# homenc/HElib

Measured on AMD Instinct MI355X. Metric: ctxt_x_ctxt_mults_per_sec_incl_relinearize, higher is better.
Workload: dtype u64; 1 GPU; BGV m=32768 p=65537 bits=950 (L=16x60b, K=6x56b, 6 small primes, D=3): Ctxt::multiplyBy on FRESH ciphertexts = multLowLvl (bringToSet x2 + tensorProduct) + reLinearize (dropSmallAndSpecialPrimes + key switch), benchmarks/bgv_basic.cpp:144-165; added noise MEASURED as in the reference (device canonical-embedding norms, read back lazily); the loop is driven by the C++17 host (libhelib_amd_host.so); ; batch_per_gpu=128, pairs_all_ranks=128

## Files before the change

### helib_amd/csrc/engine.hip

```cpp
#include <hip/hip_runtime.h>

#include <cstdarg>
#include <cstdio>
#include <cstdlib>
#include <cstring>
#include <algorithm>
#include <chrono>
#include <map>
#include <mutex>
#include <string>
#include <unordered_set>
#include <vector>

#include "../../include/helib_amd.h"
#include "arena.h"
#include "prof.h"
#include "switches.h"
#include "dev_common.h"
#include "hostmath.h"
#include "bluestein.h"
#include "pfa_dev.h"
#include "rns_kernels.h"
#include "mfma_ext.h"
#include "rns_mfma_dev.h"
#include "norm_kernels.h"
#include "prg_kernels.h"

namespace hx {
hipError_t launch_ntt_pow2(int logn, bool inverse, const uint64_t* in, uint64_t* out,
                           const NttRows& rows, int nrows, int batch, const PrimeDev* primes,
                           const TW* tw_arena, hipStream_t st);
hipError_t launch_ntt_pow2_lazy_in(int logn, const uint64_t* in, uint64_t* out, const NttRows& rows, int nrows, int batch,
                                   const PrimeDev* primes, const TW* tw_arena, hipStream_t st);
hipError_t launch_keyswitch_last_pow2(int logn, int nd, const KsLastArgs& A, const RowMap2& map, const KsLastPlan& plan, int device,
                                      const PrimeDev* primes, const TW* tw_arena, hipStream_t st);
hipError_t launch_ntt_half15_fwd(bool lazy_in, const uint64_t* in, uint64_t* out, const NttRows& rows, int nrows, int batch,
                                 const PrimeDev* sub_primes, const TW* tw_arena, hipStream_t st);
hipError_t launch_moddown_pow2(int logn, const PolyBases& data, const PolyBases& out, int drop_row,
                               int drop_prime, const NttRows& keep, int nkeep, int batch,
                               const ModDownPrep& P, const ModDownApply& A, const PrimeDev* primes,
                               const TW* tw_arena, hipStream_t st);
hipError_t launch_moddown_prep_pow2(int logn, const PolyBases& polys, int drop_row, int drop_prime, int batch,
                                    const ModDownPrep& P, const PrimeDev* primes, const TW* tw_arena,
                                    hipStream_t st);
hipError_t launch_moddown_prep_multi_pow2(int logn, const PolyBases& polys, const PrepMulti& M, int ndrop, int batch,
                                          const ModDownPrep& P, const PrimeDev* primes, const TW* tw_arena,
                                          hipStream_t st);
hipError_t launch_moddown_apply_plain_pow2(int logn, const PolyBases& polys, const PolyBases& outs,
                                           const NttRows& keep, int nkeep, int batch, const ModDownApply& A,
                                           const PrimeDev* primes, const TW* tw_arena, hipStream_t st);
hipError_t launch_moddown_prep_multi_tensor_pow2(int logn, const TensorSrc& T, const PrepMulti& M, int ndrop, int batch,
                                                 const ModDownPrep& P, const PrimeDev* primes, const TW* tw_arena,
                                                 hipStream_t st);
hipError_t launch_moddown_apply_plain_tensor_pow2(int logn, const TensorSrc& T, const PolyBases& outs, const NttRows& keep,
                                                  int nkeep, int batch, const ModDownApply& A, const PrimeDev* primes,
                                                  const TW* tw_arena, hipStream_t st);
hipError_t launch_moddown_tensor_pow2(int logn, const TensorSrc& T, const PolyBases& outs, int drop_row, int drop_prime,
                                      const NttRows& keep, int nkeep, int batch, const ModDownPrep& P,
                                      const ModDownApply& A, const PrimeDev* primes, const TW* tw_arena, hipStream_t st);
hipError_t launch_ntt_inv_mul_pow2(int logn, const uint64_t* a, const uint64_t* b, uint64_t* out, const NttRows& rows,
                                   int nrows, int batch, const PrimeDev* primes, const TW* tw_arena, hipStream_t st);
hipError_t launch_conv_rows(int logn, const ConvRowArgs& A, const ConvRows& R, int nunits, const PrimeDev* cprimes,
                            const TW* tw_arena, hipStream_t st);
}

using hx::ExtArgs;
using hx::ExtPlanDev;
using hx::MAX_ROWS;
static constexpr int MAX_EXT_SRC = hx::EXT_MAXSRC;
using hx::ModDownApply;
using hx::ModDownPrep;
using hx::NttRows;
using hx::PolyBases;
using hx::PrimeDev;
using hx::RowMap;
using hx::RowMap2;
using hx::RowScalars;
using hx::TW;

static thread_local std::string g_err;
static int fail(int code, const char* fmt, ...)
{
  char buf[512];
  va_list ap;
  va_start(ap, fmt);
  vsnprintf(buf, sizeof buf, fmt, ap);
  va_end(ap);
  g_err = buf;
  return code;
}
#define HIPCHK(expr)                                                                     \
  do {                                                                                   \
    hipError_t _e = (expr);                                                              \
    if (_e != hipSuccess) {                                                              \
      (void)hipGetLastError();  \
      return fail(HX_ERR_DEVICE, "%s failed: %s (%s:%d)", #expr, hipGetErrorString(_e),  \
                  __FILE__, __LINE__);                                                   \
    }                                                                                    \
  } while (0)
#define CHK(expr)          \
  do {                     \
// ... 4306 lines not shown
    plan.fd[r] = (uint16_t)fd[r];
  }
  hx::KsLastArgs A;
  CHK(ks_fix_table(c, all, owner, digit_primes, &A.fix));
  A.dig_in = dig_in;
  A.dig_ev = dig_ev;
  A.kb = W->d_b;
  A.ka = W->d_a;
  A.out0 = out0;
  A.out1 = out1;
  A.own_src = own_src;
  A.acc0 = t0s ? t0s : out0;
  A.acc1 = t0s ? t1s : out1;
  A.scale_parts = t0s ? 1 : 0;
  A.nall = nall;
  A.wrows = (int)W->row_idx.size();
  A.batch = batch;
  hipError_t e = hx::launch_keyswitch_last_pow2(c->logn, ndig, A, map, plan, c->device, c->d_primes, c->d_tw, c->stream);
  if (e != hipSuccess)
    return fail(HX_ERR_DEVICE, "key-switch launch failed: %s", hipGetErrorString(e));
  return HX_OK;
}

extern "C" int hx_key_switch_digits(const hx_poly* digits, const hx_ksk* W, hx_poly* out0,
                                    hx_poly* out1)
{
  if (!digits || !W || !out0 || !out1)
    return fail(HX_ERR_INVALID, "null argument");
  hx_ctx* c = digits->ctx;
  CTX_ENTER(c);
  const int nall = out0->nrows();
  if (nall == 0 || out1->prime_idx != out0->prime_idx || out0->batch != digits->batch ||
      out1->batch != digits->batch)
    return fail(HX_ERR_PRIMESET, "Ctxt::addPart: ctxt has primes not in part");
  if (digits->nrows() % nall != 0 || digits->nrows() / nall > W->ndig || digits->nrows() == 0)
    return fail(HX_ERR_INVALID, "W must have as many columns as there are digits");
  const int ndig = digits->nrows() / nall;
  for (int d = 0; d < ndig; d++)
    for (int r = 0; r < nall; r++)
      if (digits->prime_idx[(size_t)d * nall + r] != out0->prime_idx[r])
        return fail(HX_ERR_PRIMESET, "digit rows do not match the ciphertext's primes");
  OWN(out0);
  OWN(out1);
  return keyswitch_launch(c, digits->d, W, out0->prime_idx, digits->batch, out0->d, out1->d, nall,
                          nullptr, nullptr, nullptr, ndig);
}

static int relin_core(hx_ctx* c, const uint64_t* t2e, const std::vector<int>& own,
                      const std::vector<int>& all, const hx_ksk* W, const int* dig_idx,
                      const int* dig_off, int ndig, int batch, uint64_t* out0, uint64_t* out1,
                      const uint64_t* t0s = nullptr, const uint64_t* t1s = nullptr, const hx::TensorSrc* ts = nullptr)
{
  const int L = (int)own.size(), nall = (int)all.size();
  const size_t rw = (size_t)batch * c->phim;
  CHK(ensure_scratch(c, 2, (size_t)L * rw));
  if (ts) {
    NttRows nr;
    for (int r = 0; r < L; r++) {
      nr.row[r] = (uint16_t)r;
      nr.prime[r] = (uint16_t)own[r];
    }
    hipError_t e = hx::launch_ntt_inv_mul_pow2(c->logn, ts->a1, ts->b1, c->scratch[2], nr, L, batch, c->d_primes,
                                               c->d_tw, c->stream);
    if (e != hipSuccess)
      return fail(HX_ERR_DEVICE, "NTT launch failed: %s", hipGetErrorString(e));
  } else {
    std::vector<std::pair<int, int>> rows;
    for (int r = 0; r < L; r++)
      rows.emplace_back(r, own[r]);
    CHK(ntt_list(c, t2e, c->scratch[2], rows, batch, true));
  }
  CHK(ensure_scratch(c, 1, (size_t)ndig * nall * rw));
  std::vector<int> owner;
  {
    int rc = break_digits_fused(c, c->scratch[2], own, dig_idx, dig_off, ndig, all, c->scratch[1],
                                rw, &owner, digits_lazy_ok(c));
    if (rc == HX_ERR_UNSUPPORTED)
      rc = break_digits_coef(c, c->scratch[2], own, dig_idx, dig_off, ndig, all, c->scratch[1], rw,
                             false, &owner);
    if (rc != HX_OK)
      return rc;
  }
  uint64_t* digits_eval = c->scratch[1];
  const bool fuse_last = !ts && ks_last_ok(c, W, all, owner, L, ndig);
  const std::vector<int> fd = fuse_last ? ks_last_digit(owner, ndig) : std::vector<int>(nall, -1);
  {
    std::vector<std::pair<int, int>> rows;
    for (int d = 0; d < ndig; d++)
      for (int r = 0; r < nall; r++)
        if (owner[r] != d && fd[r] != d)
          rows.emplace_back(d * nall + r, all[r]);
    if (c->pow2 && c->logn == 15 && c->sw.half15) {
      CHK(ensure_scratch(c, 10, (size_t)ndig * nall * rw));
      digits_eval = c->scratch[10];
    }
    CHK(ntt_list(c, c->scratch[1], digits_eval, rows, batch, false, true));
  }
  std::vector<std::vector<int>> dprimes(ndig);
  for (int d = 0; d < ndig; d++)
    dprimes[d].assign(dig_idx + dig_off[d], dig_idx + dig_off[d + 1]);
  if (fuse_last)
    return keyswitch_last_launch(c, c->scratch[1], digits_eval, W, all, batch, out0, out1, t2e, owner, dprimes, ndig, t0s, t1s);
  return keyswitch_launch(c, digits_eval, W, all, batch, out0, out1, L, t2e, &owner, &dprimes, ndig,
                          t0s, t1s, ts);
}

static std::vector<uint64_t> special_factor(hx_ctx* c, const std::vector<int>& own, const int* sp,
                                            int nsp)
{
  std::vector<uint64_t> f(own.size());
  for (size_t r = 0; r < own.size(); r++) {
    uint64_t q = c->primes[own[r]].q, v = 1;
    for (int s = 0; s < nsp; s++)
      v = hxh::mulmod(v, c->primes[sp[s]].q % q, q);
    f[r] = v;
  }
  return f;
}

extern "C" int hx_mul_relin(const hx_poly* c0, const hx_poly* c1, const hx_poly* d0,
                            const hx_poly* d1, const hx_ksk* W, const int* dig_idx,
                            const int* dig_off, int ndig, hx_poly* out0, hx_poly* out1)
{
  if (!c0 || !c1 || !d0 || !d1 || !W || !out0 || !out1 || !dig_idx || !dig_off)
    return fail(HX_ERR_INVALID, "null argument");
  hx_ctx* c = c0->ctx;
  CTX_ENTER(c);
  if (ndig > W->ndig || ndig < 1)
    return fail(HX_ERR_INVALID, "W must have as many columns as there are digits");
  int L = c0->nrows(), nall = (int)W->row_idx.size(), K = nall - L;
  if (K < 0)
    return fail(HX_ERR_PRIMESET, "key-switching matrix has fewer primes than the ciphertext");
  for (int r = 0; r < L; r++)
    if (W->row_idx[r] != c0->prime_idx[r])
      return fail(HX_ERR_PRIMESET, "key-switching matrix rows must start with the ctxt primes");
  if (out0->batch != c0->batch || out1->batch != c0->batch || out0->ctx != c || out1->ctx != c)
    return fail(HX_ERR_INVALID, "Context mismatch");
  {
    const hx_poly* ops4[4] = {c0, c1, d0, d1};
    for (auto* p : ops4)
      if (p->ctx != c || p->batch != c0->batch || p->prime_idx != c0->prime_idx)
        return fail(HX_ERR_PRIMESET, "tensorProduct: parts must be defined relative to the same set of primes");
  }
  size_t rw = c0->row_words();
  OWN(out0);
  OWN(out1);
  CHK(poly_reserve(out0, nall, out0 == c0 || out0 == c1 || out0 == d0 || out0 == d1));
  CHK(poly_reserve(out1, nall, out1 == c0 || out1 == c1 || out1 == d0 || out1 == d1));
  out0->prime_idx = W->row_idx;
  out1->prime_idx = W->row_idx;
  const bool fuse_off = c->sw.no_mulrelin_fuse;
  const hx_poly* ins[4] = {c0, c1, d0, d1};
  bool alias = false;
  for (auto* p : ins)
    alias = alias || p == out0 || p == out1 || p->d == out0->d || p->d == out1->d;
  if (!fuse_off && !alias && c->pow2 && c->logn >= 13 && c->logn <= 15 && L <= MAX_ROWS) {
    hx::TensorSrc T{c0->d, c1->d, d0->d, d1->d};
    return relin_core(c, nullptr, c0->prime_idx, W->row_idx, W, dig_idx, dig_off, ndig, c0->batch, out0->d, out1->d,
                      nullptr, nullptr, &T);
  }
  CHK(ensure_scratch(c, 0, (size_t)L * rw));
  std::vector<uint64_t> f = special_factor(c, c0->prime_idx, W->row_idx.data() + L, K);
  CHK(tensor_launch(c0, c1, d0, d1, out0->d, out1->d, c->scratch[0], f.data()));
  return relin_core(c, c->scratch[0], c0->prime_idx, W->row_idx, W, dig_idx, dig_off, ndig,
                    c0->batch, out0->d, out1->d);
}

// ... 226 lines not shown
```

### helib_amd/csrc/ntt_kernels.hip

```cpp
#include <cstdlib>
#include "dev_common.h"
#include "prof.h"

#include "ntt_kernel_util.h"

#ifdef HX_NTT_ONLY
#define HX_SFX2(n, s) n##_L##s
#define HX_SFX1(n, s) HX_SFX2(n, s)
#define HX_ENTRY(n) HX_SFX1(n, HX_NTT_ONLY)
#else
#define HX_ENTRY(n) n
#endif
#if !defined(HX_NTT_ONLY) || HX_NTT_ONLY == 13
#define HX_SZ_13(...) case 13: return __VA_ARGS__;
#else
#define HX_SZ_13(...)
#endif
#if !defined(HX_NTT_ONLY) || HX_NTT_ONLY == 14
#define HX_SZ_14(...) case 14: return __VA_ARGS__;
#else
#define HX_SZ_14(...)
#endif
#if !defined(HX_NTT_ONLY) || HX_NTT_ONLY == 15
#define HX_SZ_15(...) case 15: return __VA_ARGS__;
// ... 640 lines not shown
    });
  }
  template <int LOGN, class AR, int B, bool EST>
  __device__ __forceinline__ void store_all(unsigned tid, uint64_t (&v)[32], const QC& qc, StorePrefetch&) const
  {
    if (part == 1)
      store_part<LOGN, AR, B, EST, true>(tid, v, qc);
    else
      store_part<LOGN, AR, B, EST, false>(tid, v, qc);
  }
  __device__ __forceinline__ void put(unsigned tid, unsigned c, uint64_t o) const
  {
    asm volatile("buffer_store_dwordx2 %0, %1, %2, %3 offen" HX_NT_ASM
                 :
                 : "v"(o), "v"((int)(tid * 8u)), "s"(ro), "s"((int)(c * 8u))
                 : "memory");
  }
  __device__ __forceinline__ TW last_tw(TW def, int) const { return def; }
  __device__ __forceinline__ TWM last_tw(TWM def, int) const { return def; }
};
template <int LOGN, bool PLAIN>
__global__ void __launch_bounds__(Geo<LOGN>::T, HX_NTT_MINWAVES(LOGN))
ntt_moddown_apply_tensor_kernel(TensorSrc T, PolyBases outs, NttRows rows, int nkeep, int batch, ModDownApply A,
                                const PrimeDev* __restrict__ primes, const TW* __restrict__ tw_arena)
{
  extern __shared__ __attribute__((aligned(16))) uint32_t lds[];
  const MdWork Wk = md_work(blockIdx.x, (unsigned)nkeep, 3u * (unsigned)batch);
  if (!Wk.active)
    return;
  const unsigned ri = Wk.ri, pb = Wk.pb;
#ifdef HX_TENSOR_PARTS_APART
  const int b = (int)(pb % (unsigned)batch);
  const unsigned pi = pb / (unsigned)batch;
#else
  const int b = (int)(pb / 3u);
  const unsigned pi = pb % 3u;
#endif
  const PrimeDev* pd = primes + uniform_u16(rows.prime, ri);
  const size_t N = Geo<LOGN>::N;
  const ModDownRow R = A.rows[ri];
  uint64_t* odata = poly_base(outs, pi);
  const size_t eoff = ((size_t)pi * batch + b) * N;
  const uint64_t* xrow = PLAIN ? A.delta + (size_t)pi * (size_t)A.delta_poly_stride + ((size_t)ri * batch + b) * N
                               : A.xs + eoff;
  const ModDownTensorIO<PLAIN> io(xrow, PLAIN ? nullptr : A.S + eoff, R, T, pi,
                                  ((size_t)uniform_u16(rows.row, ri) * batch + b) * N, R.mode != 2,
                                  odata + ((size_t)R.out_row * batch + b) * N, (unsigned)N * 8u, pd);
  ntt_body<LOGN, false>(lds, io, tw_arena + pd->tw_fwd_off, pd);
}

template <int LOGN, bool INV, int LB = 1>
__global__ void __launch_bounds__(Geo<LOGN>::T, HX_NTT_MINWAVES(LOGN))
ntt_row_kernel(const uint64_t* in, uint64_t* out, NttRows rows, int batch,
               const PrimeDev* __restrict__ primes, const TW* __restrict__ tw_arena)
{
  extern __shared__ __attribute__((aligned(16))) uint32_t lds[];
  const unsigned wid = xcd_remap(blockIdx.x, gridDim.x);
  const unsigned ri = wid / (unsigned)batch;
  const int b = (int)(wid % (unsigned)batch);
  const int row = (int)uniform_u16(rows.row, ri);
  const PrimeDev* pd = primes + uniform_u16(rows.prime, ri);
  const size_t roff = ((size_t)row * batch + b) * (size_t)Geo<LOGN>::N;
  const TW* tw = tw_arena + (INV ? pd->tw_inv_off : pd->tw_fwd_off);

#ifdef HX_NTT_PTRIO
  const PtrIO io{in + roff, out + roff};
#else
  const BufIOT<LB> io(in + roff, out + roff, (unsigned)Geo<LOGN>::N * 8u);
#endif
  ntt_body<LOGN, INV>(lds, io, tw, pd);
}

#if !defined(HX_NTT_PART) || HX_NTT_PART == 2
template <int ND>
struct KsLastIO {
  static constexpr int LOAD_BOUND = 8;
#ifndef HX_DIGITS_LB8
  template <class AR>
  static constexpr int load_bound() { return AR::PROTH ? 2 : 8; }
#endif
  static constexpr bool LAZY_STORE = true;
  static constexpr bool PIPELINED = false;
  static constexpr int DEPTH = ND <= 2 ? 2 : 1;
  static constexpr bool SPLIT = ND >= 4;
  struct StorePrefetch {};
  v4i32 rin;
  const KsLastArgs& A;
  unsigned row, b, brow, fd;
  int owner;
  uint64_t q, mu63, mu64;
  uint32_t k;
  TW ps;
  TW pinv[ND - 1];
  __device__ KsLastIO(const KsLastArgs& A_, unsigned row_, unsigned b_, unsigned brow_, unsigned fd_, unsigned bytes,
                      const PrimeDev* pd)
      : rin(make_rsrc(A_.dig_in + (((size_t)fd_ * (size_t)A_.nall + row_) * (size_t)A_.batch + b_) * (size_t)(bytes / 8u), bytes)),
        A(A_), row(row_), b(b_), brow(brow_), fd(fd_), q(pd->q), mu63(pd->mu63), mu64(pd->mu64), k(pd->k)
  {
    ro_u64 fw = as_ro(reinterpret_cast<const uint64_t*>(A_.fix + row_));
    constexpr unsigned PINV = offsetof(KsFix, pinv) / 8u, PSC = offsetof(KsFix, pscale) / 8u;
    owner = (int)(int64_t)fw[0];
    ps.w = A_.scale_parts ? fw[PSC] : 1;
    ps.wp = A_.scale_parts ? fw[PSC + 1] : mu64;
#pragma unroll
    for (int e = 0; e < ND - 1; e++) {
      const bool in = e < owner;
      pinv[e].w = in ? fw[PINV + 2 * e] : 1;
      pinv[e].wp = in ? fw[PINV + 2 * e + 1] : mu64;
    }
  }
  __device__ __forceinline__ uint64_t load(unsigned tid, unsigned c) const
  {
    v2i32 r = hx_buffer_load_v2(rin, (int)(tid * 8u), (int)(c * 8u), HX_NT);
    return ((uint64_t)(uint32_t)r.y << 32) | (uint32_t)r.x;
  }
  template <int LOGN>
  __device__ __forceinline__ void store_prefetch(unsigned, StorePrefetch&) const {}
  template <bool NT>
  static __device__ __forceinline__ uint64_t ld_pinned(const v4i32& r, unsigned tid, int soff)
  {
    uint64_t x;
    if constexpr (NT)
      asm volatile("buffer_load_dwordx2 %0, %1, %2, %3 offen" HX_NT_ASM : "=v"(x) : "v"((int)(tid * 8u)), "s"(r), "s"(soff) : "memory");
    else
      asm volatile("buffer_load_dwordx2 %0, %1, %2, %3 offen" : "=v"(x) : "v"((int)(tid * 8u)), "s"(r), "s"(soff) : "memory");
    return x;
  }
  static __device__ __forceinline__ void put(const v4i32& r, unsigned tid, unsigned c, uint64_t o)
  {
    asm volatile("buffer_store_dwordx2 %0, %1, %2, %3 offen" HX_NT_ASM : : "v"(o), "v"((int)(tid * 8u)), "s"(r), "s"((int)(c * 8u)) : "memory");
  }
#define HX_KV(i) "+v"(x[i])
#define HX_KS_WAIT(NW, ...)                                                                \
  template <int N>                                                                         \
  static __device__ __forceinline__ void pinned_wait(uint64_t (&x)[NW])                    \
  {                                                                                        \
    asm volatile("s_waitcnt vmcnt(%" #NW ")" : __VA_ARGS__ : "n"(N) : "memory");           \
  }
  HX_KS_WAIT(4, HX_KV(0), HX_KV(1), HX_KV(2), HX_KV(3))
  HX_KS_WAIT(5, HX_KV(0), HX_KV(1), HX_KV(2), HX_KV(3), HX_KV(4))
  HX_KS_WAIT(7, HX_KV(0), HX_KV(1), HX_KV(2), HX_KV(3), HX_KV(4), HX_KV(5), HX_KV(6))
  HX_KS_WAIT(9, HX_KV(0), HX_KV(1), HX_KV(2), HX_KV(3), HX_KV(4), HX_KV(5), HX_KV(6), HX_KV(7), HX_KV(8))
  HX_KS_WAIT(8, HX_KV(0), HX_KV(1), HX_KV(2), HX_KV(3), HX_KV(4), HX_KV(5), HX_KV(6), HX_KV(7))
  HX_KS_WAIT(10, HX_KV(0), HX_KV(1), HX_KV(2), HX_KV(3), HX_KV(4), HX_KV(5), HX_KV(6), HX_KV(7), HX_KV(8), HX_KV(9))
  HX_KS_WAIT(11, HX_KV(0), HX_KV(1), HX_KV(2), HX_KV(3), HX_KV(4), HX_KV(5), HX_KV(6), HX_KV(7), HX_KV(8), HX_KV(9), HX_KV(10))
  HX_KS_WAIT(13, HX_KV(0), HX_KV(1), HX_KV(2), HX_KV(3), HX_KV(4), HX_KV(5), HX_KV(6), HX_KV(7), HX_KV(8), HX_KV(9), HX_KV(10),
             HX_KV(11), HX_KV(12))
#undef HX_KS_WAIT
#undef HX_KV
  template <int LOGN, class AR, int B, bool OWNED>
  __device__ __forceinline__ void store_rows(unsigned tid, uint64_t (&v)[32], const QC& qc) const
  {
    constexpr int NMEM = OWNED ? ND - 2 : ND - 1, NACC = OWNED ? 3 : 0, NW = NMEM + NACC + (SPLIT ? ND : 2 * ND);
    constexpr int KB0 = NMEM + NACC, KA0 = KB0 + ND;
    constexpr size_t N = Geo<LOGN>::N;
    constexpr unsigned bytes = (unsigned)N * 8u;
    const size_t eoff = ((size_t)row * (size_t)A.batch + b) * N;
    const size_t dstride = (size_t)A.nall * (size_t)A.batch * N;
    const unsigned kstride = (unsigned)A.wrows * bytes;
    v4i32 rm[NMEM > 0 ? NMEM : 1];
    int kd[ND];
#pragma unroll
    for (int s = 0; s < NMEM; s++) {
      const unsigned d = (OWNED && s >= owner) ? (unsigned)s + 1u : (unsigned)s;
      rm[s] = make_rsrc(A.dig_ev + (size_t)d * dstride + eoff, bytes);
      kd[s] = (int)(d * kstride);
    }
    kd[NMEM] = (int)(fd * kstride);
    if constexpr (OWNED)
      kd[NMEM + 1] = (int)((unsigned)owner * kstride);
    const v4i32 rkb = make_rsrc(A.kb + (size_t)brow * N, (unsigned)(ND - 1) * kstride + bytes);
    const v4i32 rka = make_rsrc(A.ka + (size_t)brow * N, (unsigned)(ND - 1) * kstride + bytes);
    const v4i32 ro0 = make_rsrc(A.out0 + eoff, bytes), ro1 = make_rsrc(A.out1 + eoff, bytes);
    const v4i32 rown = make_rsrc(OWNED ? A.own_src + eoff : A.out0 + eoff, bytes);
    const v4i32 ra0 = make_rsrc(OWNED ? A.acc0 + eoff : A.out0 + eoff, bytes);
    const v4i32 ra1 = make_rsrc(OWNED ? (A.acc1 ? A.acc1 : A.acc0) + eoff : A.out0 + eoff, bytes);
    const uint64_t m1 = A.acc1 ? ~(uint64_t)0 : 0;
    uint32_t cm[NMEM > 0 ? NMEM : 1];
#pragma unroll
    for (int s = 0; s < NMEM; s++)
      cm[s] = s < owner ? ~0u : 0u;
    const uint32_t cmf = (owner == ND - 1) ? ~0u : 0u;
    auto masked = [](uint64_t x, uint32_t m) { return ((uint64_t)((uint32_t)(x >> 32) & m) << 32) | ((uint32_t)x & m); };
    auto request = [&](auto I, uint64_t (&w)[NW]) {
      constexpr int i = decltype(I)::value;
      const int c8 = (int)(eval_const<LOGN>(i) * 8u);
      static_for<0, NMEM>([&](auto S) { w[decltype(S)::value] = ld_pinned<true>(rm[decltype(S)::value], tid, c8); });
      if constexpr (OWNED) {
        w[NMEM] = ld_pinned<true>(rown, tid, c8);
        w[NMEM + 1] = ld_pinned<true>(ra0, tid, c8);
        w[NMEM + 2] = ld_pinned<true>(ra1, tid, c8);
      }
      static_for<0, ND>([&](auto S) { w[KB0 + decltype(S)::value] = ld_pinned<false>(rkb, tid, kd[decltype(S)::value] + c8); });
      if constexpr (!SPLIT)
        static_for<0, ND>([&](auto S) { w[KA0 + decltype(S)::value] = ld_pinned<false>(rka, tid, kd[decltype(S)::value] + c8); });
    };
    uint64_t wb[DEPTH][NW];
    uint64_t k2[ND];
    request(std::integral_constant<int, 0>{}, wb[0]);
    static_for<0, 32>([&](auto II) {
      constexpr int i = decltype(II)::value;
      constexpr bool more = i + 1 < 32;
      uint64_t(&w)[NW] = wb[DEPTH == 2 ? (i & 1) : 0];
      if constexpr (DEPTH == 2) {
        if constexpr (more)
          request(std::integral_constant<int, i + 1>{}, wb[(i + 1) & 1]);
        pinned_wait<(i > 0 ? 2 : 0) + (more ? NW : 0)>(w);
      } else {
        pinned_wait<(i > 0 ? (SPLIT ? 1 : 2) : 0)>(w);
      }
      const uint64_t xf = norm_from<B, true>(v[i], qc);
      const unsigned c = eval_const<LOGN>(i);
      uint64_t x[ND];
      static_for<0, NMEM>([&](auto S) { x[decltype(S)::value] = w[decltype(S)::value]; });
      x[NMEM] = xf;
      u128 s0 = 0, s1 = 0;
      if constexpr (OWNED) {
        uint64_t own = w[NMEM];
        static_for<0, NMEM>([&](auto S) {
          constexpr int s = decltype(S)::value;
          own = mul_shoup(own + q - masked(w[s], cm[s]), pinv[s].w, pinv[s].wp, q);
        });
        x[NMEM + 1] = mul_shoup(own + q - masked(xf, cmf), pinv[ND - 2].w, pinv[ND - 2].wp, q);
        s0 = mul_shoup(w[NMEM + 1], ps.w, ps.wp, q);
        s1 = mul_shoup(w[NMEM + 2], ps.w, ps.wp, q) & m1;
      }
      static_for<0, ND>([&](auto S) { s0 += (u128)x[decltype(S)::value] * w[KB0 + decltype(S)::value]; });
      if constexpr (SPLIT) {
        const int c8 = (int)(c * 8u);
        static_for<0, ND>([&](auto S) { k2[decltype(S)::value] = ld_pinned<false>(rka, tid, kd[decltype(S)::value] + c8); });
        put(ro0, tid, c, tensor_red128(s0, q, mu63, k));
        pinned_wait<1>(k2);
        static_for<0, ND>([&](auto S) { s1 += (u128)x[decltype(S)::value] * k2[decltype(S)::value]; });
        if constexpr (more)
          request(std::integral_constant<int, i + 1>{}, wb[0]);
        put(ro1, tid, c, tensor_red128(s1, q, mu63, k));
      } else {
        static_for<0, ND>([&](auto S) { s1 += (u128)x[decltype(S)::value] * w[KA0 + decltype(S)::value]; });
        if constexpr (DEPTH == 1 && more)
          request(std::integral_constant<int, i + 1>{}, wb[0]);
        put(ro0, tid, c, tensor_red128(s0, q, mu63, k));
        put(ro1, tid, c, tensor_red128(s1, q, mu63, k));
      }
      HX_SCHED_FENCE();
    });
  }
  template <int LOGN, class AR, int B, bool EST>
  __device__ __forceinline__ void store_all(unsigned tid, uint64_t (&v)[32], const QC& qc, StorePrefetch&) const
  {
    if constexpr (EST) {
      if (owner >= 0)
        store_rows<LOGN, AR, B, true>(tid, v, qc);
      else
        store_rows<LOGN, AR, B, false>(tid, v, qc);
    }
  }
  __device__ __forceinline__ TW last_tw(TW def, int) const { return def; }
  __device__ __forceinline__ TWM last_tw(TWM def, int) const { return def; }
};
template <int LOGN, int ND>
__global__ void __launch_bounds__(Geo<LOGN>::T, HX_NTT_MINWAVES(LOGN))
ntt_keyswitch_last_kernel(KsLastArgs A, RowMap2 map, KsLastPlan plan, const PrimeDev* __restrict__ primes,
                          const TW* __restrict__ tw_arena)
{
  extern __shared__ __attribute__((aligned(16))) uint32_t lds[];
  const KsWork W = ks_last_work(blockIdx.x, (unsigned)A.nall, (unsigned)A.batch);
  const PrimeDev* pd = primes + uniform_u16(map.p, W.row);
  const KsLastIO<ND> io(A, W.row, W.b, uniform_u16(map.brow, W.row), uniform_u16(plan.fd, W.row), (unsigned)Geo<LOGN>::N * 8u, pd);
  ntt_body<LOGN, false>(lds, io, tw_arena + pd->tw_fwd_off, pd);
}
template <int LOGN, int ND>
static hipError_t launch_ks_last(const KsLastArgs& A, const RowMap2& map, const KsLastPlan& plan, int device,
                                 const PrimeDev* primes, const TW* tw_arena, hipStream_t st)
{
  constexpr size_t lds_bytes = (size_t)Geo<LOGN>::LDS_WORDS * 4;
  hipError_t e = hxp::dyn_lds((const void*)ntt_keyswitch_last_kernel<LOGN, ND>, (int)lds_bytes, device);
  if (e != hipSuccess)
    return e;
  HX_LAUNCH((ntt_keyswitch_last_kernel<LOGN, ND>), dim3((unsigned)A.nall * (unsigned)A.batch), dim3(Geo<LOGN>::T), lds_bytes,
            st, A, map, plan, primes, tw_arena);
  return hipGetLastError();
}
template <int LOGN>
static hipError_t launch_ks_last_nd(int nd, const KsLastArgs& A, const RowMap2& map, const KsLastPlan& plan, int device,
                                    const PrimeDev* primes, const TW* tw_arena, hipStream_t st)
{
  switch (nd) {
    case 2: return launch_ks_last<LOGN, 2>(A, map, plan, device, primes, tw_arena, st);
    case 3: return launch_ks_last<LOGN, 3>(A, map, plan, device, primes, tw_arena, st);
    case 4: return launch_ks_last<LOGN, 4>(A, map, plan, device, primes, tw_arena, st);
  }
  return hipErrorInvalidValue;
}
hipError_t HX_ENTRY(launch_keyswitch_last_pow2)(int logn, int nd, const KsLastArgs& A, const RowMap2& map, const KsLastPlan& plan,
                                                int device, const PrimeDev* primes, const TW* tw_arena, hipStream_t st)
{
  switch (logn) {
    HX_SZ(13, launch_ks_last_nd<13>(nd, A, map, plan, device, primes, tw_arena, st))
    HX_SZ(14, launch_ks_last_nd<14>(nd, A, map, plan, device, primes, tw_arena, st))
    HX_SZ(15, launch_ks_last_nd<15>(nd, A, map, plan, device, primes, tw_arena, st))
  }
  return hipErrorInvalidValue;
}
#endif

#if !defined(HX_NTT_PART) || HX_NTT_PART == 1
template <bool PROTH>
struct MulLoadIO {
  static constexpr int LOAD_BOUND = 1;
  static constexpr bool LAZY_STORE = false;
  static constexpr bool PIPELINED = false;
  template <class AR>
  static constexpr int inv_load_bound() { return PROTH ? 2 : 1; }
  struct StorePrefetch {};
  v4i32 ra, rb, ro;
  uint64_t q, mu63, r2;
  uint32_t k;
  __device__ MulLoadIO(const uint64_t* a_row, const uint64_t* b_row, uint64_t* o_row, unsigned bytes, const PrimeDev* pd)
      : ra(make_rsrc(a_row, bytes)), rb(make_rsrc(b_row, bytes)), ro(make_rsrc(o_row, bytes)), q(pd->q), mu63(pd->mu63),
        r2(pd->r2), k(pd->k)
  {
  }
  __device__ __forceinline__ uint64_t load(unsigned tid, unsigned c) const
  {
    const v2i32 x = hx_buffer_load_v2(ra, (int)(tid * 8u), (int)(c * 8u), HX_NT);
    const v2i32 y = hx_buffer_load_v2(rb, (int)(tid * 8u), (int)(c * 8u), HX_NT);
    const uint64_t a = ((uint64_t)(uint32_t)x.y << 32) | (uint32_t)x.x, b = ((uint64_t)(uint32_t)y.y << 32) | (uint32_t)y.x;
    const u128 p = (u128)a * b;
// ... 502 lines not shown
```

### helib_amd/csrc/work_map.h

```cpp
#pragma once

#if defined(__HIPCC__)
#define HXW __host__ __device__ __forceinline__
#else
#define HXW inline
#endif

namespace hx {

HXW unsigned xcd_remap_id(unsigned id, unsigned nwg)
{
  const unsigned xcd = id & 7u, slot = id >> 3, qd = nwg >> 3, r = nwg & 7u;
  return (xcd < r ? xcd * (qd + 1) : r * (qd + 1) + (xcd - r) * qd) + slot;
}

struct MdTile {
  unsigned g, rg, chunk, per_xcd;
};
HXW MdTile md_tile(unsigned nkeep, unsigned npb)
{
  MdTile t;
  t.g = 1;
  while (t.g < 8 && (nkeep + t.g - 1) / t.g > 8)
    t.g *= 2;
  t.rg = (nkeep + t.g - 1) / t.g;
  const unsigned xpg = 8 / t.g;
  t.chunk = (npb + xpg - 1) / xpg;
  t.per_xcd = t.rg * t.chunk;
  return t;
}
struct MdWork {
  bool active;
  unsigned ri, pb;
};
HXW MdWork md_work(unsigned block, unsigned nkeep, unsigned npb)
{
  const MdTile T = md_tile(nkeep, npb);
  const unsigned xcd = block & 7u, slot = block >> 3;
  const unsigned grp = xcd % T.g, part = xcd / T.g;
  const unsigned r0 = grp * T.rg, pb0 = part * T.chunk;
  const unsigned nr = r0 < nkeep ? (T.rg < nkeep - r0 ? T.rg : nkeep - r0) : 0u;
  const unsigned nloc = pb0 < npb ? (T.chunk < npb - pb0 ? T.chunk : npb - pb0) : 0u;
  MdWork w;
  w.active = slot < nr * nloc;
  w.ri = w.active ? r0 + slot % nr : 0u;
  w.pb = w.active ? pb0 + slot / nr : 0u;
  return w;
}

struct KsWork {
  unsigned row, b;
};
HXW KsWork ks_last_work(unsigned block, unsigned nrows, unsigned batch)
{
  const unsigned w = xcd_remap_id(block, nrows * batch);
  KsWork k;
  k.row = w / batch;
  k.b = w % batch;
  return k;
}

}
```

Measured before the change: 44660 mult/s.

## Split ND=3 fused keyswitch loads into two staggered half-pipelines and rebuild rsrcs lazily

For three digits, the fused last-NTT keyswitch kernel now issues loads in two groups: digits, owner and acc0 with key B, then acc1 with key A. Each output half is computed and stored while the other group's loads for the next column are in flight. Buffer resources are kept as uniform 64-bit bases and rebuilt at each use, which cuts SGPR pressure. A host-side guard disables fusion when the key span could overflow a 32-bit buffer offset, which also works as a correctness check.

```diff
diff --git a/helib_amd/csrc/engine.hip b/helib_amd/csrc/engine.hip
--- a/helib_amd/csrc/engine.hip
+++ b/helib_amd/csrc/engine.hip
@@ -17,6 +17,7 @@
 #include "prof.h"
 #include "switches.h"
 #include "dev_common.h"
+#include "work_map.h"
 #include "hostmath.h"
 #include "bluestein.h"
 #include "pfa_dev.h"
@@ -4489,7 +4490,7 @@
       return rc;
   }
   uint64_t* digits_eval = c->scratch[1];
-  const bool fuse_last = !ts && ks_last_ok(c, W, all, owner, L, ndig);
+  const bool fuse_last = !ts && ks_last_ok(c, W, all, owner, L, ndig) && hx::ks_key_span_ok((size_t)ndig, W->row_idx.size(), c->phim);
   const std::vector<int> fd = fuse_last ? ks_last_digit(owner, ndig) : std::vector<int>(nall, -1);
   {
     std::vector<std::pair<int, int>> rows;
diff --git a/helib_amd/csrc/ntt_kernels.hip b/helib_amd/csrc/ntt_kernels.hip
--- a/helib_amd/csrc/ntt_kernels.hip
+++ b/helib_amd/csrc/ntt_kernels.hip
@@ -746,6 +746,7 @@
   static constexpr bool LAZY_STORE = true;
   static constexpr bool PIPELINED = false;
   static constexpr int DEPTH = ND <= 2 ? 2 : 1;
+  static constexpr bool HALF = ND == 3;
   static constexpr bool SPLIT = ND >= 4;
   struct StorePrefetch {};
   v4i32 rin;
@@ -780,9 +781,26 @@
   }
   template <int LOGN>
   __device__ __forceinline__ void store_prefetch(unsigned, StorePrefetch&) const {}
+  static __device__ __forceinline__ uint64_t row_base(const uint64_t* p)
+  {
+    const uint64_t a = (uint64_t)p;
+    return ((uint64_t)(uint32_t)__builtin_amdgcn_readfirstlane((int)(uint32_t)(a >> 32)) << 32) |
+           (uint32_t)__builtin_amdgcn_readfirstlane((int)(uint32_t)a);
+  }
+  static __device__ __forceinline__ v4i32 rsrc_at(uint64_t base, unsigned bytes)
+  {
+    asm volatile("" : "+s"(base));
+    v4i32 r;
+    r.x = (int)(uint32_t)base;
+    r.y = (int)(uint32_t)(base >> 32);
+    r.z = (int)bytes;
+    r.w = 0x00020000;
+    return r;
+  }
   template <bool NT>
-  static __device__ __forceinline__ uint64_t ld_pinned(const v4i32& r, unsigned tid, int soff)
-  {
+  static __device__ __forceinline__ uint64_t ld_pinned(uint64_t base, unsigned bytes, unsigned tid, int soff)
+  {
+    const v4i32 r = rsrc_at(base, bytes);
     uint64_t x;
     if constexpr (NT)
       asm volatile("buffer_load_dwordx2 %0, %1, %2, %3 offen" HX_NT_ASM : "=v"(x) : "v"((int)(tid * 8u)), "s"(r), "s"(soff) : "memory");
@@ -790,8 +808,9 @@
       asm volatile("buffer_load_dwordx2 %0, %1, %2, %3 offen" : "=v"(x) : "v"((int)(tid * 8u)), "s"(r), "s"(soff) : "memory");
     return x;
   }
-  static __device__ __forceinline__ void put(const v4i32& r, unsigned tid, unsigned c, uint64_t o)
-  {
+  static __device__ __forceinline__ void put(uint64_t base, unsigned bytes, unsigned tid, unsigned c, uint64_t o)
+  {
+    const v4i32 r = rsrc_at(base, bytes);
     asm volatile("buffer_store_dwordx2 %0, %1, %2, %3 offen" HX_NT_ASM : : "v"(o), "v"((int)(tid * 8u)), "s"(r), "s"((int)(c * 8u)) : "memory");
   }
 #define HX_KV(i) "+v"(x[i])
@@ -801,8 +820,10 @@
   {                                                                                        \
     asm volatile("s_waitcnt vmcnt(%" #NW ")" : __VA_ARGS__ : "n"(N) : "memory");           \
   }
+  HX_KS_WAIT(3, HX_KV(0), HX_KV(1), HX_KV(2))
   HX_KS_WAIT(4, HX_KV(0), HX_KV(1), HX_KV(2), HX_KV(3))
   HX_KS_WAIT(5, HX_KV(0), HX_KV(1), HX_KV(2), HX_KV(3), HX_KV(4))
+  HX_KS_WAIT(6, HX_KV(0), HX_KV(1), HX_KV(2), HX_KV(3), HX_KV(4), HX_KV(5))
   HX_KS_WAIT(7, HX_KV(0), HX_KV(1), HX_KV(2), HX_KV(3), HX_KV(4), HX_KV(5), HX_KV(6))
   HX_KS_WAIT(9, HX_KV(0), HX_KV(1), HX_KV(2), HX_KV(3), HX_KV(4), HX_KV(5), HX_KV(6), HX_KV(7), HX_KV(8))
   HX_KS_WAIT(8, HX_KV(0), HX_KV(1), HX_KV(2), HX_KV(3), HX_KV(4), HX_KV(5), HX_KV(6), HX_KV(7))
@@ -822,92 +843,143 @@
     const size_t eoff = ((size_t)row * (size_t)A.batch + b) * N;
     const size_t dstride = (size_t)A.nall * (size_t)A.batch * N;
     const unsigned kstride = (unsigned)A.wrows * bytes;
-    v4i32 rm[NMEM > 0 ? NMEM : 1];
+    uint64_t bm[NMEM > 0 ? NMEM : 1];
     int kd[ND];
 #pragma unroll
     for (int s = 0; s < NMEM; s++) {
       const unsigned d = (OWNED && s >= owner) ? (unsigned)s + 1u : (unsigned)s;
-      rm[s] = make_rsrc(A.dig_ev + (size_t)d * dstride + eoff, bytes);
+      bm[s] = row_base(A.dig_ev + (size_t)d * dstride + eoff);
       kd[s] = (int)(d * kstride);
     }
     kd[NMEM] = (int)(fd * kstride);
     if constexpr (OWNED)
       kd[NMEM + 1] = (int)((unsigned)owner * kstride);
-    const v4i32 rkb = make_rsrc(A.kb + (size_t)brow * N, (unsigned)(ND - 1) * kstride + bytes);
-    const v4i32 rka = make_rsrc(A.ka + (size_t)brow * N, (unsigned)(ND - 1) * kstride + bytes);
-    const v4i32 ro0 = make_rsrc(A.out0 + eoff, bytes), ro1 = make_rsrc(A.out1 + eoff, bytes);
-    const v4i32 rown = make_rsrc(OWNED ? A.own_src + eoff : A.out0 + eoff, bytes);
-    const v4i32 ra0 = make_rsrc(OWNED ? A.acc0 + eoff : A.out0 + eoff, bytes);
-    const v4i32 ra1 = make_rsrc(OWNED ? (A.acc1 ? A.acc1 : A.acc0) + eoff : A.out0 + eoff, bytes);
-    const uint64_t m1 = A.acc1 ? ~(uint64_t)0 : 0;
+    const unsigned kbytes = (unsigned)(ND - 1) * kstride + bytes;
+    const uint64_t bkb = row_base(A.kb + (size_t)brow * N), bka = row_base(A.ka + (size_t)brow * N);
+    const uint64_t bo0 = row_base(A.out0 + eoff), bo1 = row_base(A.out1 + eoff);
+    const uint64_t bown = row_base(OWNED ? A.own_src + eoff : A.out0 + eoff);
+    const uint64_t ba0 = row_base(OWNED ? A.acc0 + eoff : A.out0 + eoff);
+    const uint64_t ba1 = row_base(OWNED ? (A.acc1 ? A.acc1 : A.acc0) + eoff : A.out0 + eoff);
+    const uint32_t m1 = A.acc1 ? ~0u : 0u;
     uint32_t cm[NMEM > 0 ? NMEM : 1];
 #pragma unroll
     for (int s = 0; s < NMEM; s++)
       cm[s] = s < owner ? ~0u : 0u;
     const uint32_t cmf = (owner == ND - 1) ? ~0u : 0u;
     auto masked = [](uint64_t x, uint32_t m) { return ((uint64_t)((uint32_t)(x >> 32) & m) << 32) | ((uint32_t)x & m); };
-    auto request = [&](auto I, uint64_t (&w)[NW]) {
+    auto digits_of = [&](auto I, const uint64_t* m, uint64_t own, uint64_t (&x)[ND]) {
       constexpr int i = decltype(I)::value;
-      const int c8 = (int)(eval_const<LOGN>(i) * 8u);
-      static_for<0, NMEM>([&](auto S) { w[decltype(S)::value] = ld_pinned<true>(rm[decltype(S)::value], tid, c8); });
+      const uint64_t xf = norm_from<B, true>(v[i], qc);
+      static_for<0, NMEM>([&](auto S) { x[decltype(S)::value] = m[decltype(S)::value]; });
+      x[NMEM] = xf;
       if constexpr (OWNED) {
-        w[NMEM] = ld_pinned<true>(rown, tid, c8);
-        w[NMEM + 1] = ld_pinned<true>(ra0, tid, c8);
-        w[NMEM + 2] = ld_pinned<true>(ra1, tid, c8);
-      }
-      static_for<0, ND>([&](auto S) { w[KB0 + decltype(S)::value] = ld_pinned<false>(rkb, tid, kd[decltype(S)::value] + c8); });
-      if constexpr (!SPLIT)
-        static_for<0, ND>([&](auto S) { w[KA0 + decltype(S)::value] = ld_pinned<false>(rka, tid, kd[decltype(S)::value] + c8); });
-    };
-    uint64_t wb[DEPTH][NW];
-    uint64_t k2[ND];
-    request(std::integral_constant<int, 0>{}, wb[0]);
-    static_for<0, 32>([&](auto II) {
-      constexpr int i = decltype(II)::value;
-      constexpr bool more = i + 1 < 32;
-      uint64_t(&w)[NW] = wb[DEPTH == 2 ? (i & 1) : 0];
-      if constexpr (DEPTH == 2) {
-        if constexpr (more)
-          request(std::integral_constant<int, i + 1>{}, wb[(i + 1) & 1]);
-        pinned_wait<(i > 0 ? 2 : 0) + (more ? NW : 0)>(w);
-      } else {
-        pinned_wait<(i > 0 ? (SPLIT ? 1 : 2) : 0)>(w);
-      }
-      const uint64_t xf = norm_from<B, true>(v[i], qc);
-      const unsigned c = eval_const<LOGN>(i);
-      uint64_t x[ND];
-      static_for<0, NMEM>([&](auto S) { x[decltype(S)::value] = w[decltype(S)::value]; });
-      x[NMEM] = xf;
-      u128 s0 = 0, s1 = 0;
-      if constexpr (OWNED) {
-        uint64_t own = w[NMEM];
         static_for<0, NMEM>([&](auto S) {
           constexpr int s = decltype(S)::value;
-          own = mul_shoup(own + q - masked(w[s], cm[s]), pinv[s].w, pinv[s].wp, q);
+          own = mul_shoup(own + q - masked(m[s], cm[s]), pinv[s].w, pinv[s].wp, q);
         });
         x[NMEM + 1] = mul_shoup(own + q - masked(xf, cmf), pinv[ND - 2].w, pinv[ND - 2].wp, q);
-        s0 = mul_shoup(w[NMEM + 1], ps.w, ps.wp, q);
-        s1 = mul_shoup(w[NMEM + 2], ps.w, ps.wp, q) & m1;
       }
-      static_for<0, ND>([&](auto S) { s0 += (u128)x[decltype(S)::value] * w[KB0 + decltype(S)::value]; });
-      if constexpr (SPLIT) {
-        const int c8 = (int)(c * 8u);
-        static_for<0, ND>([&](auto S) { k2[decltype(S)::value] = ld_pinned<false>(rka, tid, kd[decltype(S)::value] + c8); });
-        put(ro0, tid, c, tensor_red128(s0, q, mu63, k));
-        pinned_wait<1>(k2);
-        static_for<0, ND>([&](auto S) { s1 += (u128)x[decltype(S)::value] * k2[decltype(S)::value]; });
+    };
+    if constexpr (HALF) {
+      constexpr int NH0 = NMEM + (OWNED ? 2 : 0) + ND, NH1 = (OWNED ? 1 : 0) + ND, K0 = NH0 - ND, K1 = NH1 - ND;
+      auto request0 = [&](auto I, uint64_t (&h)[NH0]) {
+        const int c8 = (int)(eval_const<LOGN>(decltype(I)::value) * 8u);
+        static_for<0, NMEM>([&](auto S) { h[decltype(S)::value] = ld_pinned<true>(bm[decltype(S)::value], bytes, tid, c8); });
+        if constexpr (OWNED) {
+          h[NMEM] = ld_pinned<true>(bown, bytes, tid, c8);
+          h[NMEM + 1] = ld_pinned<true>(ba0, bytes, tid, c8);
+        }
+        static_for<0, ND>([&](auto S) { h[K0 + decltype(S)::value] = ld_pinned<false>(bkb, kbytes, tid, kd[decltype(S)::value] + c8); });
+      };
+      auto request1 = [&](auto I, uint64_t (&h)[NH1]) {
+        const int c8 = (int)(eval_const<LOGN>(decltype(I)::value) * 8u);
+        if constexpr (OWNED)
+          h[0] = ld_pinned<true>(ba1, bytes, tid, c8);
+        static_for<0, ND>([&](auto S) { h[K1 + decltype(S)::value] = ld_pinned<false>(bka, kbytes, tid, kd[decltype(S)::value] + c8); });
+      };
+      uint64_t h0[NH0], h1[NH1];
+      request0(std::integral_constant<int, 0>{}, h0);
+      request1(std::integral_constant<int, 0>{}, h1);
+      static_for<0, 32>([&](auto II) {
+        constexpr int i = decltype(II)::value;
+        constexpr bool more = i + 1 < 32;
+        const unsigned c = eval_const<LOGN>(i);
+        pinned_wait<(i > 0 ? 2 : 0) + NH1>(h0);
+        uint64_t x[ND];
+        digits_of(II, h0, OWNED ? h0[NMEM] : 0, x);
+        u128 s0 = 0;
+        if constexpr (OWNED)
+          s0 = mul_shoup(h0[NMEM + 1], ps.w, ps.wp, q);
+        static_for<0, ND>([&](auto S) { s0 += (u128)x[decltype(S)::value] * h0[K0 + decltype(S)::value]; });
         if constexpr (more)
-          request(std::integral_constant<int, i + 1>{}, wb[0]);
-        put(ro1, tid, c, tensor_red128(s1, q, mu63, k));
-      } else {
-        static_for<0, ND>([&](auto S) { s1 += (u128)x[decltype(S)::value] * w[KA0 + decltype(S)::value]; });
-        if constexpr (DEPTH == 1 && more)
-          request(std::integral_constant<int, i + 1>{}, wb[0]);
-        put(ro0, tid, c, tensor_red128(s0, q, mu63, k));
-        put(ro1, tid, c, tensor_red128(s1, q, mu63, k));
-      }
-      HX_SCHED_FENCE();
-    });
+          request0(std::integral_constant<int, i + 1>{}, h0);
+        put(bo0, bytes, tid, c, tensor_red128(s0, q, mu63, k));
+        pinned_wait<(i > 0 ? 2 : 1) + (more ? NH0 : 0)>(h1);
+        u128 s1 = 0;
+        if constexpr (OWNED)
+          s1 = masked(mul_shoup(h1[0], ps.w, ps.wp, q), m1);
+        static_for<0, ND>([&](auto S) { s1 += (u128)x[decltype(S)::value] * h1[K1 + decltype(S)::value]; });
+        if constexpr (more)
+          request1(std::integral_constant<int, i + 1>{}, h1);
+        put(bo1, bytes, tid, c, tensor_red128(s1, q, mu63, k));
+        HX_SCHED_FENCE();
+      });
+    } else {
+      auto request = [&](auto I, uint64_t (&w)[NW]) {
+        constexpr int i = decltype(I)::value;
+        const int c8 = (int)(eval_const<LOGN>(i) * 8u);
+        static_for<0, NMEM>([&](auto S) { w[decltype(S)::value] = ld_pinned<true>(bm[decltype(S)::value], bytes, tid, c8); });
+        if constexpr (OWNED) {
+          w[NMEM] = ld_pinned<true>(bown, bytes, tid, c8);
+          w[NMEM + 1] = ld_pinned<true>(ba0, bytes, tid, c8);
+          w[NMEM + 2] = ld_pinned<true>(ba1, bytes, tid, c8);
+        }
+        static_for<0, ND>([&](auto S) { w[KB0 + decltype(S)::value] = ld_pinned<false>(bkb, kbytes, tid, kd[decltype(S)::value] + c8); });
+        if constexpr (!SPLIT)
+          static_for<0, ND>([&](auto S) { w[KA0 + decltype(S)::value] = ld_pinned<false>(bka, kbytes, tid, kd[decltype(S)::value] + c8); });
+      };
+      uint64_t wb[DEPTH][NW];
+      uint64_t k2[ND];
+      request(std::integral_constant<int, 0>{}, wb[0]);
+      static_for<0, 32>([&](auto II) {
+        constexpr int i = decltype(II)::value;
+        constexpr bool more = i + 1 < 32;
+        uint64_t(&w)[NW] = wb[DEPTH == 2 ? (i & 1) : 0];
+        if constexpr (DEPTH == 2) {
+          if constexpr (more)
+            request(std::integral_constant<int, i + 1>{}, wb[(i + 1) & 1]);
+          pinned_wait<(i > 0 ? 2 : 0) + (more ? NW : 0)>(w);
+        } else {
+          pinned_wait<(i > 0 ? (SPLIT ? 1 : 2) : 0)>(w);
+        }
+        const unsigned c = eval_const<LOGN>(i);
+        uint64_t x[ND];
+        digits_of(II, w, OWNED ? w[NMEM] : 0, x);
+        u128 s0 = 0, s1 = 0;
+        if constexpr (OWNED) {
+          s0 = mul_shoup(w[NMEM + 1], ps.w, ps.wp, q);
+          s1 = masked(mul_shoup(w[NMEM + 2], ps.w, ps.wp, q), m1);
+        }
+        static_for<0, ND>([&](auto S) { s0 += (u128)x[decltype(S)::value] * w[KB0 + decltype(S)::value]; });
+        if constexpr (SPLIT) {
+          const int c8 = (int)(c * 8u);
+          static_for<0, ND>([&](auto S) { k2[decltype(S)::value] = ld_pinned<false>(bka, kbytes, tid, kd[decltype(S)::value] + c8); });
+          put(bo0, bytes, tid, c, tensor_red128(s0, q, mu63, k));
+          pinned_wait<1>(k2);
+          static_for<0, ND>([&](auto S) { s1 += (u128)x[decltype(S)::value] * k2[decltype(S)::value]; });
+          if constexpr (more)
+            request(std::integral_constant<int, i + 1>{}, wb[0]);
+          put(bo1, bytes, tid, c, tensor_red128(s1, q, mu63, k));
+        } else {
+          static_for<0, ND>([&](auto S) { s1 += (u128)x[decltype(S)::value] * w[KA0 + decltype(S)::value]; });
+          if constexpr (DEPTH == 1 && more)
+            request(std::integral_constant<int, i + 1>{}, wb[0]);
+          put(bo0, bytes, tid, c, tensor_red128(s0, q, mu63, k));
+          put(bo1, bytes, tid, c, tensor_red128(s1, q, mu63, k));
+        }
+        HX_SCHED_FENCE();
+      });
+    }
   }
   template <int LOGN, class AR, int B, bool EST>
   __device__ __forceinline__ void store_all(unsigned tid, uint64_t (&v)[32], const QC& qc, StorePrefetch&) const
diff --git a/helib_amd/csrc/work_map.h b/helib_amd/csrc/work_map.h
--- a/helib_amd/csrc/work_map.h
+++ b/helib_amd/csrc/work_map.h
@@ -60,4 +60,10 @@
   return k;
 }
 
+HXW bool ks_key_span_ok(unsigned long long ndig, unsigned long long wrows, unsigned long long n)
+{
+  return ndig >= 1 && ndig <= 64 && wrows <= (1ull << 20) && n <= (1ull << 20) &&
+         (ndig - 1) * wrows * n * 8ull + n * 8ull < (1ull << 31);
 }
+
+}
```

New measurement: 44810 mult/s (median of 6 runs). About the same (+0.3%).
